# sunchao/leveldb-rs

Hardware: AMD Instinct MI355X
Metric: GiB/s device-resident batched CRC32C, 4KiB blocks; %HBM-peak at 1/2/4/8 GPUs (higher is better)
Workload: dtype u32

## Files before the change

leveldb-rs_amd/csrc/blocks.hip:

```cpp
#include <hip/hip_runtime.h>

#include <algorithm>
#include <string>

#include "lvh.h"

namespace lvk {

template <int G, bool STRIDED>
__global__ __launch_bounds__(kThreads) void crc32c_batch_kernel(Params P, const uint4 *__restrict__ image) {
    if (static_cast<uint64_t>(blockIdx.x) * kWaves * (64 / G) >= P.n) return;
    stage_tables(image);
    const uint32_t lane = threadIdx.x & 63u;
    const uint32_t wave = threadIdx.x >> 6;
    const Lut L = make_lut(lane);
    constexpr uint32_t kGroups = 64 / G;
    const uint64_t gid = (static_cast<uint64_t>(blockIdx.x) * kWaves + wave) * kGroups + lane / G;
    const uint64_t gstride = static_cast<uint64_t>(gridDim.x) * kWaves * kGroups;
    group_stream<G, STRIDED>(P, gid, gstride, lane % G, L);
}

constexpr uint32_t kFuseMax = 16;

__device__ __forceinline__ void fuse_pieces(const Params &P, const uint32_t *fm, uint32_t (&res)[kWaves][64],
                                            uint32_t lane, uint32_t wave) {
    __syncthreads();
    if (wave != 0) return;
    const uint32_t s = 1u << P.pshift;
    const uint64_t v = static_cast<uint64_t>(blockIdx.x) * 64u + lane;
    const uint32_t k = lane & (s - 1u);
    uint32_t acc = v < P.n ? gf2_apply(fm + (s - 1u - k) * 33u, res[lane >> 2][lane & 3u]) : 0u;
    for (uint32_t d = s >> 1; d >= 1; d >>= 1) acc ^= __shfl_xor(acc, d);
    if (v < P.n && k == 0) P.out[v >> P.pshift] = final_crc(P, acc);
}
static_assert(kFuseMax * 33 <= kWaves * 64, "fused combine matrices fit g_oidx");
template <int G, bool SEEDED, bool PIECES = false, bool FUSE = false, bool GATHER = false>
__global__ __launch_bounds__(kThreads) void crc32c_blocks_kernel(Params P, uint32_t nb,
                                                                 const uint4 *__restrict__ image) {
    static_assert(!FUSE || (PIECES && G == 16), "fused combine: pieces of the G = 16 kernel");
    const uint32_t lane = threadIdx.x & 63u;
    const uint32_t wave = __builtin_amdgcn_readfirstlane(threadIdx.x >> 6);
    constexpr uint32_t kGroups = 64 / G;
    constexpr uint64_t kRow = 16ull * G;
    constexpr uint64_t kBatch = kRow * U;
    const uint32_t gl = lane % G;
    constexpr uint32_t kW = kWaves;
    uint64_t blk = (static_cast<uint64_t>(blockIdx.x) * kW + wave) * kGroups + lane / G;
    const uint64_t gstride = static_cast<uint64_t>(gridDim.x) * kW * kGroups;
    const uint64_t wblk0 = (static_cast<uint64_t>(blockIdx.x) * kW + wave) * kGroups;
    const uint64_t pmask = (1ull << P.pshift) - 1;
    auto block_off = [&](uint64_t k) -> uint64_t {
        const uint64_t kk = k < P.n ? k : 0;
        const uint64_t b = PIECES ? kk >> P.pshift : kk;
        if constexpr (GATHER) return P.off[b];
        return b * P.stride;
    };
    auto report = [&](uint32_t bad) {
        if constexpr (GATHER)
            if (bad && P.herr) atomicOr(P.herr, bad);
    };
    auto block_at = [&](uint64_t k, uint64_t bo) {
        const uint64_t kk = k < P.n ? k : 0;
        if constexpr (GATHER) bo &= ~static_cast<uint64_t>(15);
        if constexpr (PIECES) return P.base + bo + (kk & pmask) * P.plen + 16u * gl;
        return P.base + bo + 16u * gl;
    };
    auto block_ptr = [&](uint64_t k) { return block_at(k, block_off(k)); };
    auto seed_ld = [&](uint64_t k) -> uint32_t {
        const uint64_t kk = k < P.n ? k : 0;
        if constexpr (PIECES) {
            const uint32_t sd = SEEDED ? ~P.seed[kk >> P.pshift] : 0xffffffffu;
            return (kk & pmask) ? 0u : sd;
        }
        return ~P.seed[kk];
    };
    constexpr bool kVarS0 = SEEDED || PIECES;

    const uint64_t o0 = block_off(blk);
    uint64_t ptr = block_at(blk, o0);
    uint64_t o1 = GATHER ? block_off(blk + gstride) : 0;
    uint64_t o2 = o1;
    uint32_t s0 = kVarS0 ? seed_ld(blk) : 0xffffffffu;
    uint32_t s0n = s0;
    uint4 slot0[U], slot1[U];
#pragma unroll
    for (uint32_t i = 0; i < U; ++i) slot0[i] = load16(ptr + kRow * i);
    const uint64_t nblk = PIECES ? (P.n >> P.pshift) : P.n;
    const uint64_t lstr = static_cast<uint64_t>(gridDim.x) * kThreads;
    const uint64_t lb0 = static_cast<uint64_t>(blockIdx.x) * kThreads + threadIdx.x;
    uint32_t lq[4] = {0, 0, 0, 0};
    const bool lcheck = GATHER && P.herr;
    if (lcheck) {
#pragma unroll
        for (uint32_t i = 0; i < 4; ++i) {
            const uint64_t b = lb0 + i * lstr;
            lq[i] = b < nblk ? P.len[b] ^ P.hlen : 0u;
        }
    }
    uint32_t *const fm = &g_oidx[0][0];
    if constexpr (FUSE) {
        const uint32_t nw = (1u << P.pshift) * 32u;
        for (uint32_t i = threadIdx.x; i < nw; i += kThreads) fm[(i >> 5) * 33 + (i & 31u)] = P.mats[i];
    }
    stage_tables(image);
    uint32_t lbad = lq[0] | lq[1] | lq[2] | lq[3];
    if (lcheck)
        for (uint64_t b = lb0 + 4 * lstr; b < nblk; b += lstr) lbad |= P.len[b] ^ P.hlen;
    if constexpr (GATHER) report(((o0 & 15u) ? LV_HINT_ERR_MISALIGNED : 0u) | (lbad ? LV_HINT_ERR_NOT_UNIFORM : 0u));
    if (wblk0 >= P.n) {
        if constexpr (FUSE) fuse_pieces(P, fm, g_ocrc, lane, wave);
        return;
    }
    if constexpr (PIECES) {
        if (nb <= U && (FUSE || wblk0 + gstride >= P.n)) {
            uint4 v1[U], v2[U], v3[U];
#pragma unroll
            for (uint32_t i = 0; i < U; ++i) {
                v1[i] = load16(ptr + kBatch * (nb > 1 ? 1u : 0u) + kRow * i);
                v2[i] = load16(ptr + kBatch * (nb > 2 ? 2u : 0u) + kRow * i);
                v3[i] = load16(ptr + kBatch * (nb > 3 ? 3u : 0u) + kRow * i);
            }
            const Lut L = make_lut(lane);
            uint32_t A[U];
            if (gl == 0) slot0[0].x ^= kVarS0 ? seed_ld(blk) : 0xffffffffu;
            fold_batch<true>(slot0, A, L);
            if (nb > 1) fold_batch<false>(v1, A, L);
            if (nb > 2) fold_batch<false>(v2, A, L);
            if (nb > 3) fold_batch<false>(v3, A, L);
            const uint32_t X = merge_group<G, -1, -1, true>(A, L);
            if constexpr (FUSE) {
                if (gl == 0) g_ocrc[wave][lane / G] = X;
                fuse_pieces(P, fm, g_ocrc, lane, wave);
            } else {
                if (gl == 0 && blk < P.n) P.out[blk] = X;
            }
            return;
        }
    }
    const uint64_t rounds = (P.n - 1 - wblk0) / gstride + 1;
    if (G == 16 && nb >= 8 && rounds * nb >= 64)
        for (uint32_t k = 0; k < wave * LVK_STAGGER; ++k) __builtin_amdgcn_s_sleep(32);
    const Lut L = make_lut(lane);
    uint32_t A[U];
    uint32_t st_val = 0;
    uint64_t st_ptr = 0;

    auto step = [&](uint64_t r, uint32_t j, uint4(&cur)[U], uint4(&nxt)[U]) {
        const bool lastj = j + 1 == nb;
        const bool more = !lastj || r + 1 < rounds;
        if constexpr (GATHER) o2 = block_off(blk + 2 * gstride);
        const uint64_t nptr = lastj ? (GATHER ? block_at(blk + gstride, o1) : block_ptr(blk + gstride)) : ptr + kBatch;
        const uint64_t lptr = more ? nptr : GATHER ? ptr : P.base + 16u * gl;
        if constexpr (kVarS0) s0n = seed_ld(blk + gstride);
#pragma unroll
        for (uint32_t i = 0; i < U; ++i) nxt[i] = load16(lptr + kRow * i);
        if (j == 0) {
            if (gl == 0) cur[0].x ^= s0;
            fold_batch<true>(cur, A, L);
        } else {
            fold_batch<false>(cur, A, L);
        }
        if (lastj) {
            const uint32_t X = merge_group<G, -1, -1, true>(A, L);
            if (gl == 0) g_ocrc[wave][(r % G) * kGroups + lane / G] = PIECES ? X : final_crc(P, X);
            if (!FUSE && ((r + 1) % G == 0 || r + 1 == rounds)) {
                __builtin_amdgcn_wave_barrier();
                const uint64_t r0 = r - r % G;
                const uint64_t k = wblk0 + (r0 + lane / kGroups) * gstride + lane % kGroups;
                st_val = g_ocrc[wave][lane];
                st_ptr = reinterpret_cast<uint64_t>(P.out + (k < P.n ? k : 0));
                if (lane < (r - r0 + 1) * kGroups && k < P.n) *reinterpret_cast<uint32_t *>(st_ptr) = st_val;
                __builtin_amdgcn_wave_barrier();
            }
            blk += gstride;
            if constexpr (kVarS0) s0 = s0n;
            if constexpr (GATHER) {
                if (o1 & 15u) report(LV_HINT_ERR_MISALIGNED);
                o1 = o2;
            }
        }
        ptr = nptr;
    };

    const uint64_t total = rounds * nb;
    uint64_t t = 0;
    uint64_t r = 0;
    uint32_t j = 0;
    for (;;) {
        step(r, j, slot0, slot1);
        if (++t == total) break;
        if (++j == nb) { j = 0; ++r; }
        step(r, j, slot1, slot0);
        if (++t == total) break;
        if (++j == nb) { j = 0; ++r; }
    }
    asm volatile("" ::"v"(st_val), "v"(st_ptr));
    if constexpr (FUSE) fuse_pieces(P, fm, g_ocrc, lane, wave);
}

__global__ __launch_bounds__(256) void combine_pieces_kernel(const uint32_t *__restrict__ raw, uint64_t n, uint32_t s,
                                                             const uint32_t *__restrict__ mats,
                                                             uint32_t *__restrict__ out, uint32_t flags) {
    __shared__ uint32_t M[65 * 33];
    for (uint32_t i = threadIdx.x; i < 65 * 32; i += blockDim.x) M[(i >> 5) * 33 + (i & 31u)] = mats[i];
    __syncthreads();
    const uint32_t lane = threadIdx.x & 63u;
    const uint32_t w = s < 64 ? s : 64, reps = s <= 64 ? 1 : s / 64;
    const uint64_t nw = static_cast<uint64_t>(gridDim.x) * (blockDim.x / 64);
    for (uint64_t b = static_cast<uint64_t>(blockIdx.x) * (blockDim.x / 64) + (threadIdx.x >> 6); b < n; b += nw) {
        uint32_t acc = 0;
        if (lane < w) {
            uint32_t nx = raw[b * s + lane];
            for (uint32_t m = 0; m < reps; ++m) {
                const uint32_t cur = nx;
                if (m + 1 < reps) nx = raw[b * s + lane + 64 * (m + 1)];
                acc = (m ? gf2_apply(M + 64 * 33, acc) : 0u) ^ cur;
            }
            acc = gf2_apply(M + (w - 1 - lane) * 33, acc);
        }
#pragma unroll
        for (int k = 32; k >= 1; k >>= 1) acc ^= __shfl_xor(acc, k);
        if (lane == 0) {
            const uint32_t crc = ~acc;
            out[b] = (flags & LV_CRC_MASK) ? mask_crc(crc) : crc;
        }
    }
}

__global__ __launch_bounds__(1024) void combine_pieces_wg_kernel(const uint32_t *__restrict__ raw, uint32_t s,
                                                                 const uint32_t *__restrict__ tabs,
                                                                 uint32_t *__restrict__ out, uint32_t flags) {
    __shared__ __attribute__((aligned(16))) uint32_t T[11 * 1024];
    __shared__ uint32_t part[16];
    const uint32_t c = s / 1024u;
    const uint32_t lc = c >= 4u ? 2u : 1u;
    stage_words(T, tabs, 256u);
    stage_words(T + 1024, tabs + lc * 1024u, 10u * 256u);
    __syncthreads();
    const uint32_t t = threadIdx.x, lane = t & 63u, w = t >> 6;
    const uint64_t b = blockIdx.x;
    uint32_t acc = 0;
    for (uint32_t i = 0; i < c; ++i) acc = (i ? tab_shift(T, acc) : 0u) ^ raw[b * s + t * c + i];
#pragma unroll
    for (uint32_t u = 0; u < 6; ++u) {
        const uint32_t right = __shfl_down(acc, 1u << u);
        const uint32_t sh = tab_shift(T + (1u + u) * 1024u, acc);
        if ((lane & ((2u << u) - 1u)) == 0) acc = sh ^ right;
    }
    if (lane == 0) part[w] = acc;
    __syncthreads();
    if (w == 0) {
        acc = lane < 16u ? part[lane] : 0u;
#pragma unroll
        for (uint32_t u = 0; u < 4; ++u) {
            const uint32_t right = __shfl_down(acc, 1u << u);
            const uint32_t sh = tab_shift(T + (7u + u) * 1024u, acc);
            if ((lane & ((2u << u) - 1u)) == 0) acc = sh ^ right;
        }
        if (lane == 0) {
            const uint32_t crc = ~acc;
            out[b] = (flags & LV_CRC_MASK) ? mask_crc(crc) : crc;
        }
    }
}

}

namespace lvh {

template <int G, bool STRIDED>
void launch_one(const DevCtx &c, int gi, const uint8_t *arena, const uint64_t *off,
                const uint32_t *len, uint64_t stride, uint32_t blen, const uint32_t *seed,
                uint32_t *out, uint64_t n, uint32_t flags, hipStream_t s) {
    const uint64_t groups_per_wg = static_cast<uint64_t>(lvk::kWaves) * (64 / G);
    uint64_t grid = (n + groups_per_wg - 1) / groups_per_wg;
    if (grid > static_cast<uint64_t>(c.cus)) grid = c.cus;
    if (grid == 0) grid = 1;
    lvk::Params P{};
    P.base = reinterpret_cast<uint64_t>(arena);
    P.off = off;
    P.len = len;
    P.seed = seed;
    P.out = out;
    P.n = n;
    P.stride = stride;
    P.blen = blen;
    P.flags = flags;
    P.ent = nullptr;
    P.sseed = nullptr;
    static const std::string name = std::string("crc32c_batch_kernel<") + std::to_string(G) +
                                    (STRIDED ? ",strided>" : ",offsets>");
    g_kernel = name.c_str();
    hipLaunchKernelGGL((lvk::crc32c_batch_kernel<G, STRIDED>), dim3(static_cast<uint32_t>(grid)),
                       dim3(lvk::kThreads), 0, s, P, c.image[gi]);
}

template <bool STRIDED>
void launch_g(const DevCtx &c, int gi, const uint8_t *arena, const uint64_t *off,
              const uint32_t *len, uint64_t stride, uint32_t blen, const uint32_t *seed,
              uint32_t *out, uint64_t n, uint32_t flags, hipStream_t s) {
    switch (gi) {
        case 0: launch_one<1, STRIDED>(c, gi, arena, off, len, stride, blen, seed, out, n, flags, s); break;
        case 1: launch_one<4, STRIDED>(c, gi, arena, off, len, stride, blen, seed, out, n, flags, s); break;
        case 2: launch_one<16, STRIDED>(c, gi, arena, off, len, stride, blen, seed, out, n, flags, s); break;
        default: launch_one<64, STRIDED>(c, gi, arena, off, len, stride, blen, seed, out, n, flags, s); break;
    }
}

void launch_group(const DevCtx &c, bool strided, int gi, const uint8_t *arena, const uint64_t *off,
                  const uint32_t *len, uint64_t stride, uint32_t blen, const uint32_t *seed, uint32_t *out, uint64_t n,
                  uint32_t flags, hipStream_t s) {
    if (strided)
        launch_g<true>(c, gi, arena, off, len, stride, blen, seed, out, n, flags, s);
    else
        launch_g<false>(c, gi, arena, off, len, stride, blen, seed, out, n, flags, s);
}

uint32_t pick_split(uint64_t base, uint64_t stride, uint64_t blen, uint64_t n, int forced, int cus) {
    if (forced >= 0 || base % 16 || stride % 16) return 0;
    const uint64_t want = 4ull * static_cast<uint64_t>(cus) * lvk::kWaves;
    uint32_t ps = 0;
    while ((n << ps) < want && ps < 12) {
        const uint64_t s2 = 2ull << ps;
        if (blen % s2 || (blen / s2) % 1024 || blen / s2 < 4096) break;
        ++ps;
    }
    return ps;
}
int pick_block_gi(uint64_t base, uint64_t stride, uint64_t blen, int forced, uint64_t n, int cus) {
    if (blen == 0 || base % 16 || stride % 16) return -1;
    auto fits = [&](int gi) { return blen % (16ull * kGs[gi] * lvk::U) == 0; };
    if (forced >= 0) return fits(forced) ? forced : -1;
    if (n < 4ull * static_cast<uint64_t>(cus) * lvk::kWaves && fits(3)) return 3;
    for (int gi : {2, 1, 0})
        if (fits(gi)) return gi;
    return -1;
}

template <int G, bool GATHER>
void launch_blocks_g(const DevCtx &c, int gi, const uint8_t *base, uint64_t stride, const uint64_t *off,
                     const uint32_t *len, const HintCheck *hc, uint32_t blen, uint64_t n, const uint32_t *seed,
                     uint32_t *out, uint32_t flags, hipStream_t s) {
    const uint64_t groups_per_wg = static_cast<uint64_t>(lvk::kWaves) * (64 / G);
    uint64_t grid = (n + groups_per_wg - 1) / groups_per_wg;
    if (grid > static_cast<uint64_t>(c.cus)) grid = c.cus;
    if (grid == 0) grid = 1;
    lvk::Params P{};
    P.base = reinterpret_cast<uint64_t>(base);
    P.off = off;
    P.len = len;
    P.seed = seed;
    P.out = out;
    P.n = n;
    P.stride = stride;
    P.blen = blen;
    P.flags = flags;
    P.ent = nullptr;
    P.sseed = nullptr;
    set_hint(P, hc, blen);
    const uint32_t nb = static_cast<uint32_t>(blen / (16ull * G * lvk::U));
    static const std::string name = "crc32c_blocks_kernel<" + std::to_string(G) + (GATHER ? ",gather>" : ">");
    g_kernel = name.c_str();
    if (seed)
        hipLaunchKernelGGL((lvk::crc32c_blocks_kernel<G, true, false, false, GATHER>),
                           dim3(static_cast<uint32_t>(grid)), dim3(lvk::kThreads), 0, s, P, nb, c.image[gi]);
    else
        hipLaunchKernelGGL((lvk::crc32c_blocks_kernel<G, false, false, false, GATHER>),
                           dim3(static_cast<uint32_t>(grid)), dim3(lvk::kThreads), 0, s, P, nb, c.image[gi]);
}

template <bool GATHER>
void launch_blocks(const DevCtx &c, int gi, const uint8_t *base, uint64_t stride, const uint64_t *off,
                   const uint32_t *len, const HintCheck *hc, uint32_t blen, uint64_t n, const uint32_t *seed,
                   uint32_t *out, uint32_t flags, hipStream_t s) {
    switch (gi) {
        case 0: launch_blocks_g<1, GATHER>(c, gi, base, stride, off, len, hc, blen, n, seed, out, flags, s); break;
        case 1: launch_blocks_g<4, GATHER>(c, gi, base, stride, off, len, hc, blen, n, seed, out, flags, s); break;
        case 2: launch_blocks_g<16, GATHER>(c, gi, base, stride, off, len, hc, blen, n, seed, out, flags, s); break;
        default: launch_blocks_g<64, GATHER>(c, gi, base, stride, off, len, hc, blen, n, seed, out, flags, s); break;
    }
}

template <bool GATHER>
void launch_pieces(DevCtx &c, uint32_t ps, const uint32_t *mats, const uint32_t *tabs, const uint8_t *base,
                   uint64_t stride, const uint64_t *off, const uint32_t *len, const HintCheck *hc, uint32_t blen,
                   uint64_t n, const uint32_t *seed, uint32_t *out, uint32_t flags, hipStream_t hs, uint32_t *scr) {
    const uint64_t nv = n << ps, plen = blen >> ps;
    const uint32_t nb = static_cast<uint32_t>(plen / (16ull * 16 * lvk::U));
    lvk::Params P{};
    P.base = reinterpret_cast<uint64_t>(base);
    P.off = off;
    P.len = len;
    P.seed = seed;
    P.n = nv;
    P.stride = stride;
    P.blen = static_cast<uint32_t>(plen);
    P.flags = flags;
    P.plen = plen;
    P.pshift = ps;
    P.mats = mats;
    set_hint(P, hc, blen);
    if (!scr) {
        P.out = out;
        const dim3 grid(static_cast<uint32_t>((nv + 63) / 64));
        if (seed)
            hipLaunchKernelGGL((lvk::crc32c_blocks_kernel<16, true, true, true, GATHER>), grid, dim3(lvk::kThreads), 0,
                               hs, P, nb, c.image[2]);
        else
            hipLaunchKernelGGL((lvk::crc32c_blocks_kernel<16, false, true, true, GATHER>), grid, dim3(lvk::kThreads),
                               0, hs, P, nb, c.image[2]);
        g_kernel = GATHER ? "crc32c_blocks_kernel<16,pieces,fused,gather>" : "crc32c_blocks_kernel<16,pieces,fused>";
        return;
    }
    P.out = scr;
    const uint64_t grid = std::min<uint64_t>(c.cus, (nv + 63) / 64);
    if (seed)
        hipLaunchKernelGGL((lvk::crc32c_blocks_kernel<16, true, true, false, GATHER>), dim3(static_cast<uint32_t>(grid)),
                           dim3(lvk::kThreads), 0, hs, P, nb, c.image[2]);
    else
        hipLaunchKernelGGL((lvk::crc32c_blocks_kernel<16, false, true, false, GATHER>),
                           dim3(static_cast<uint32_t>(grid)), dim3(lvk::kThreads), 0, hs, P, nb, c.image[2]);
    if (ps >= 11) {
        hipLaunchKernelGGL(lvk::combine_pieces_wg_kernel, dim3(static_cast<uint32_t>(n)), dim3(1024), 0, hs, P.out,
                           1u << ps, tabs, out, flags);
        g_kernel = GATHER ? "crc32c_blocks_kernel<16,pieces,gather>+combine_pieces_wg_kernel"
                          : "crc32c_blocks_kernel<16,pieces>+combine_pieces_wg_kernel";
    } else {
        hipLaunchKernelGGL(lvk::combine_pieces_kernel, dim3(static_cast<uint32_t>(std::min<uint64_t>(1024, (n + 3) / 4))),
                           dim3(256), 0, hs, P.out, n, 1u << ps, mats, out, flags);
        g_kernel = GATHER ? "crc32c_blocks_kernel<16,pieces,gather>+combine_pieces_kernel"
                          : "crc32c_blocks_kernel<16,pieces>+combine_pieces_kernel";
    }
}

UniformPlan uniform_plan(int cus, uint64_t base, uint64_t stride, uint32_t blen, uint64_t n, int gi) {
    UniformPlan pl{};
    pl.ps = pick_split(base, stride, blen, n, gi, cus);
    pl.bgi = -1;
    if (pl.ps > 0) {
        const uint64_t nv = n << pl.ps;
        const bool fused = (1u << pl.ps) <= lvk::kFuseMax && nv <= 64ull * static_cast<uint64_t>(cus);
        pl.scratch = fused ? 0 : nv * 4;
    } else {
        pl.bgi = pick_block_gi(base, stride, blen, gi, n, cus);
    }
    return pl;
}

int launch_uniform(DevCtx &c, const UniformPlan &pl, const uint8_t *base, uint64_t stride, const uint64_t *off,
                   const uint32_t *len, const HintCheck *hc, uint32_t blen, uint64_t n, const uint32_t *seed,
                   uint32_t *out, uint32_t flags, hipStream_t hs, uint8_t *scr) {
    if (pl.ps > 0) {
        const uint64_t plen = blen >> pl.ps;
        const uint32_t *mats = nullptr, *tabs = nullptr;
        if (int rc = piece_mats(c, plen, &mats)) return rc;
        if (pl.scratch && pl.ps >= 11)
            if (int rc = piece_tabs(c, plen, &tabs)) return rc;
        uint32_t *s32 = pl.scratch ? reinterpret_cast<uint32_t *>(scr) : nullptr;
        if (off)
            launch_pieces<true>(c, pl.ps, mats, tabs, base, stride, off, len, hc, blen, n, seed, out, flags, hs, s32);
        else
            launch_pieces<false>(c, pl.ps, mats, tabs, base, stride, off, len, hc, blen, n, seed, out, flags, hs,
                                 s32);
        return 0;
    }
    if (off)
        launch_blocks<true>(c, pl.bgi, base, stride, off, len, hc, blen, n, seed, out, flags, hs);
    else
        launch_blocks<false>(c, pl.bgi, base, stride, off, len, hc, blen, n, seed, out, flags, hs);
    return 0;
}

}

using namespace lvh;

extern "C" {

int lv_crc32c_batch_strided(const uint8_t *d_base, uint64_t stride, uint32_t block_len, size_t n,
                            const uint32_t *d_seed, uint32_t *d_out, uint32_t flags, void *stream) {
    g_err.clear();
    if (n == 0) return LV_OK;
    if (!d_base || !d_out) return set_err(LV_ERR_INVALID, "null device pointer");
    if (n > 0xffffffffull) return set_err(LV_ERR_INVALID, "more than 2^32-1 buffers per call");
    DevCtx *c = nullptr;
    if (int rc = current_ctx(&c)) return rc;
    const int gi = forced_gi(flags);
    hipStream_t hs = static_cast<hipStream_t>(stream);
    const UniformPlan pl = uniform_plan(c->cus, reinterpret_cast<uint64_t>(d_base), stride, block_len, n, gi);
    if (pl.applies()) {
        uint8_t *scr = nullptr;
        std::unique_lock<std::mutex> ws_lk;
        if (pl.scratch)
            if (int rc = stream_ws_bytes(*c, hs, pl.scratch, &scr, &ws_lk)) return rc;
        if (int rc = launch_uniform(*c, pl, d_base, stride, nullptr, nullptr, nullptr, block_len, n, d_seed, d_out,
                                    flags, hs, scr))
            return rc;
        return check_launch();
    }
    launch_g<true>(*c, gi >= 0 ? gi : pick_gi(block_len), d_base, nullptr, nullptr, stride, block_len, d_seed,
                   d_out, n, flags, hs);
    return check_launch();
}

}
```

leveldb-rs_amd/csrc/context.hip:

```cpp
#include <hip/hip_runtime.h>

#include <algorithm>
#include <cstring>
#include <thread>

#include "../../include/lvgpu/crc32c.h"
#include "crc32c_gf2.h"
#include "lvh.h"

namespace lvk {

__device__ __forceinline__ uint64_t splitmix64(uint64_t x) {
    x += 0x9E3779B97F4A7C15ull;
    x = (x ^ (x >> 30)) * 0xBF58476D1CE4E5B9ull;
    x = (x ^ (x >> 27)) * 0x94D049BB133111EBull;
    return x ^ (x >> 31);
}

__global__ void fill_words_kernel(uint64_t *dst, uint64_t word0, uint64_t nwords, uint64_t seed) {
    for (uint64_t i = blockIdx.x * 256ull + threadIdx.x; i < nwords; i += gridDim.x * 256ull)
        dst[i] = splitmix64(seed ^ (word0 + i));
}

__global__ void fill_bytes_kernel(uint8_t *dst, uint64_t begin, uint64_t nbytes, uint64_t seed) {
    for (uint64_t i = blockIdx.x * 256ull + threadIdx.x; i < nbytes; i += gridDim.x * 256ull) {
        const uint64_t k = begin + i;
        dst[i] = static_cast<uint8_t>(splitmix64(seed ^ (k >> 3)) >> (8 * (k & 7)));
    }
}

}

namespace lvh {

thread_local std::string g_err;
thread_local const char *g_kernel = "";

int set_err(int code, const std::string &msg) {
    g_err = msg;
    return code;
}

const std::vector<uint32_t> &host_image(int gi) {
    static std::vector<uint32_t> images[kImages];
    static std::once_flag once;
    std::call_once(once, [] {
        uint32_t T[4][256], C[6][4][256];
        lvgpu::slice_tables(T);
        for (int k = 0; k < 6; ++k) lvgpu::shift_tables(16ull << k, C[k]);
        for (int i = 0; i < 4; ++i) {
            const uint64_t G = static_cast<uint64_t>(kGs[i]);
            uint32_t W4[4][256], W1[4][256], W2[4][256];
            lvgpu::shift_tables(16ull * G * lvk::U, W4);
            lvgpu::shift_tables(16ull * G, W1);
            lvgpu::shift_tables(32ull * G, W2);
            std::vector<uint32_t> &im = images[i];
            im.assign(lvk::kImageWords, 0u);
            uint32_t *ra = &im[lvk::kRegionA / 4], *rb = &im[lvk::kRegionB / 4];
            for (int e = 0; e < 256; ++e)
                for (int c = 0; c < 8; ++c)
                    for (int k = 0; k < 4; ++k) {
                        ra[e * 64 + 4 * c + k] = T[k][e];
                        ra[e * 64 + 32 + 4 * c + k] = W4[3 - k][e];
                        rb[e * 64 + 4 * c + k] = W1[3 - k][e];
                        rb[e * 64 + 32 + 4 * c + k] = W2[3 - k][e];
                    }
            uint32_t *rc = &im[lvk::kComb / 4];
            for (int k = 0; k < 6; ++k)
                for (int j = 0; j < 4; ++j)
                    for (int e = 0; e < 256; ++e) rc[(k * 4 + j) * 256 + e] = C[k][j][e];
        }
        uint32_t WT[4][256];
        lvgpu::shift_tables(256ull * lvk::kSstRows, WT);
        images[kTableImage] = images[2];
        uint32_t *ra = &images[kTableImage][lvk::kRegionA / 4];
        for (int e = 0; e < 256; ++e)
            for (int c = 0; c < 8; ++c)
                for (int k = 0; k < 4; ++k) ra[e * 64 + 32 + 4 * c + k] = WT[3 - k][e];
    });
    return images[gi];
}

DevCounters g_count[64];

DevCounters &counters() {
    int d = 0;
    if (hipGetDevice(&d) != hipSuccess || d < 0 || d >= 64) d = 0;
    return g_count[d];
}

int grow_dev(uint8_t **p, size_t *cap, size_t need) {
    if (*cap >= need) return 0;
    if (*p) LV_HIP(hipFree(*p));
    *p = nullptr;
    *cap = 0;
    LV_HIP(hipMalloc(p, need));
    counters().allocs++;
    *cap = need;
    return 0;
}

int grow_pinned(uint8_t **p, size_t *cap, size_t need) {
    if (*cap >= need) return 0;
    if (*p) LV_HIP(hipHostFree(*p));
    *p = nullptr;
    *cap = 0;
    LV_HIP(hipHostMalloc(p, need, hipHostMallocDefault));
    counters().allocs++;
    *cap = need;
    return 0;
}

bool is_pinned(const void *p) {
    hipPointerAttribute_t a;
    const hipError_t e = hipPointerGetAttributes(&a, p);
    if (e != hipSuccess) {
        (void)hipGetLastError();
        return false;
    }
    return a.type == hipMemoryTypeHost;
}

void par_memcpy(uint8_t *dst, const uint8_t *src, size_t bytes, unsigned threads) {
    unsigned nt = std::thread::hardware_concurrency();
    nt = nt == 0 ? 1 : (nt > threads ? threads : nt);
    if (bytes < (4u << 20) || nt == 1) {
        std::memcpy(dst, src, bytes);
        return;
    }
    std::vector<std::thread> th;
    const size_t per = (bytes + nt - 1) / nt;
    for (unsigned t = 0; t < nt; ++t) {
        const size_t lo = t * per;
        if (lo >= bytes) break;
        const size_t len = bytes - lo < per ? bytes - lo : per;
        th.emplace_back([=] { std::memcpy(dst + lo, src + lo, len); });
    }
    for (auto &x : th) x.join();
}

DevCtx g_dev[64];

int current_ctx(DevCtx **out) {
    int dev = 0;
    hipError_t e = hipGetDevice(&dev);
    if (e != hipSuccess) return set_err(LV_ERR_NO_DEVICE, std::string("hipGetDevice: ") + hipGetErrorString(e));
    if (dev < 0 || dev >= 64) return set_err(LV_ERR_NO_DEVICE, "device index out of range");
    DevCtx &c = g_dev[dev];
    std::lock_guard<std::mutex> lk(c.m);
    if (!c.ready) {
        hipDeviceProp_t prop;
        LV_HIP(hipGetDeviceProperties(&prop, dev));
        c.cus = prop.multiProcessorCount;
        for (int i = 0; i < kImages; ++i) {
            const auto &im = host_image(i);
            LV_HIP(hipMalloc(&c.image[i], im.size() * 4));
            counters().allocs++;
            LV_HIP(hipMemcpy(c.image[i], im.data(), im.size() * 4, hipMemcpyHostToDevice));
        }
        {
            std::vector<uint32_t> bt(lvk::kBaseMats * 1024);
            for (uint32_t i = 0; i < lvk::kBaseMats; ++i) {
                uint32_t S[4][256];
                lvgpu::shift_tables(1ull << i, S);
                for (int j = 0; j < 4; ++j)
                    for (int e = 0; e < 256; ++e) bt[i * 1024 + j * 256 + e] = S[j][e];
            }
            LV_HIP(hipMalloc(&c.base_tabs, bt.size() * 4));
            counters().allocs++;
            LV_HIP(hipMemcpy(c.base_tabs, bt.data(), bt.size() * 4, hipMemcpyHostToDevice));
        }
        c.ready = true;
    }
    *out = &c;
    return 0;
}

int pick_gi(uint64_t len) {
    if (len <= 128) return 0;
    if (len <= 1024) return 1;
    if (len <= 16384) return 2;
    return 3;
}

int forced_gi(uint32_t flags) {
    const uint32_t f = (flags & LV_CRC_GROUP_MASK) >> 8;
    return f ? static_cast<int>(f) - 1 : -1;
}

static StreamWs *find_ws(DevCtx &c, hipStream_t s, bool create) {
    std::lock_guard<std::mutex> mk(c.ws_m);
    if (!create) {
        auto it = c.ws.find(s);
        return it == c.ws.end() ? nullptr : it->second.get();
    }
    auto &slot = c.ws[s];
    if (!slot) slot.reset(new StreamWs);
    return slot.get();
}

int stream_ws_bytes(DevCtx &c, hipStream_t s, size_t need, uint8_t **out, std::unique_lock<std::mutex> *lk) {
    StreamWs *w = find_ws(c, s, true);
    *lk = std::unique_lock<std::mutex>(w->m);
    if (w->cap < need) {
        if (w->p) LV_HIP(hipFree(w->p));
        w->p = nullptr;
        w->cap = 0;
        LV_HIP(hipMalloc(&w->p, need));
        counters().allocs++;
        w->cap = need;
    }
    *out = w->p;
    return 0;
}

int stream_ws(DevCtx &c, hipStream_t s, uint64_t n, uint8_t **out, std::unique_lock<std::mutex> *lk) {
    return stream_ws_bytes(c, s, sort_ws_bytes(n), out, lk);
}

int stream_err(DevCtx &c, hipStream_t s, uint32_t **out) {
    StreamWs *w = find_ws(c, s, true);
    std::lock_guard<std::mutex> lk(w->em);
    if (!w->err) {
        LV_HIP(hipHostMalloc(reinterpret_cast<void **>(&w->herr), 4, hipHostMallocDefault));
        LV_HIP(hipMalloc(&w->err, 4));
        counters().allocs += 2;
        LV_HIP(hipMemsetAsync(w->err, 0, 4, s));
    }
    *out = w->err;
    return 0;
}
// ... 339 lines not shown
```

leveldb-rs_amd/csrc/lvh.h:

```cpp
#pragma once
#include <hip/hip_runtime.h>

#include <atomic>
#include <cstdint>
#include <map>
#include <memory>
#include <mutex>
#include <string>
#include <vector>

#include "../../include/lvgpu/crc32c.h"
#include "lv_internal.h"
#include "lvk/core.h"

namespace lvh {

extern thread_local std::string g_err;
extern thread_local const char *g_kernel;
int set_err(int code, const std::string &msg);

#define LV_HIP(call)                                                                   \
    do {                                                                               \
        hipError_t e_ = (call);                                                        \
        if (e_ != hipSuccess)                                                          \
            return set_err(static_cast<int>(e_), std::string(#call) + ": " +           \
                                                     hipGetErrorString(e_));           \
    } while (0)


constexpr int kGs[4] = {1, 4, 16, 64};
constexpr int kTableImage = 4;
constexpr uint32_t kAlRowsH = LVK_AL_ROWS;
constexpr int kAlImage = kAlRowsH == 4 ? 2 : kTableImage;
static_assert(kAlRowsH == 4 || kAlRowsH == lvk::kSstRows, "aligned rows: 4, or the table image's");
constexpr int kImages = 5;

const std::vector<uint32_t> &host_image(int gi);

struct StreamWs {
    std::mutex m;
    uint8_t *p = nullptr;
    size_t cap = 0;
    std::mutex em;
    uint32_t *err = nullptr;
    uint32_t *herr = nullptr;
};

struct DevCtx {
    std::mutex m;
    bool ready = false;
    int cus = 0;
    uint4 *image[kImages] = {};
    uint32_t *base_tabs = nullptr;
    std::mutex ws_m;
    std::map<hipStream_t, std::unique_ptr<StreamWs>> ws;
    std::mutex mats_m;
    std::map<uint64_t, uint32_t *> piece_mats;
    std::map<uint64_t, uint32_t *> piece_tabs;
    std::mutex host_m;
    uint8_t *d_arena = nullptr;
    size_t d_arena_cap = 0;
    uint8_t *d_meta = nullptr;
    size_t d_meta_cap = 0;
    uint8_t *h_meta = nullptr;
    size_t h_meta_cap = 0;
    uint8_t *h_stage[2] = {nullptr, nullptr};
    size_t h_stage_cap[2] = {0, 0};
    hipEvent_t ev[2] = {nullptr, nullptr};
    hipStream_t stream = nullptr;
    hipStream_t stream2 = nullptr;
    uint8_t *d_arena2 = nullptr;
    size_t d_arena2_cap = 0;
    uint8_t *d_scr[2] = {nullptr, nullptr};
    size_t d_scr_cap[2] = {0, 0};
    int dev = 0;
};

constexpr size_t kStageBytes = 64ull << 20;

struct DevCounters {
    std::atomic<uint64_t> h2d{0}, d2h{0}, allocs{0};
};
extern DevCounters g_count[64];
DevCounters &counters();


int grow_dev(uint8_t **p, size_t *cap, size_t need);
int grow_pinned(uint8_t **p, size_t *cap, size_t need);
bool is_pinned(const void *p);
void par_memcpy(uint8_t *dst, const uint8_t *src, size_t bytes, unsigned threads = LVK_MEMCPY_THREADS);
int current_ctx(DevCtx **out);
int pick_gi(uint64_t len);
int forced_gi(uint32_t flags);
int check_launch();

constexpr size_t al16(size_t x) { return (x + 15) & ~static_cast<size_t>(15); }

inline bool overlaps(const void *a, uint64_t ab, const void *b, uint64_t bb) {
    const uintptr_t x = reinterpret_cast<uintptr_t>(a), y = reinterpret_cast<uintptr_t>(b);
    return ab && bb && x < y + bb && y < x + ab;
}
inline bool misaligned(const void *p, uintptr_t n) { return reinterpret_cast<uintptr_t>(p) % n != 0; }

struct Carve {
    uint8_t *base;
    size_t at = 0;
    template <class T>
    T *take(size_t count) {
        const size_t o = at;
        at += al16(count * sizeof(T));
        return base ? reinterpret_cast<T *>(reinterpret_cast<uintptr_t>(base) + o) : nullptr;
    }
};

uint64_t sort_wgs(uint64_t n, uint64_t *chunk);
struct WsLayout {
    size_t m, wgb, ent, sseed, part, longs, tmp, pos, total;
};
WsLayout ws_layout(uint64_t n);
size_t sort_ws_bytes(uint64_t n);
int stream_ws_bytes(DevCtx &c, hipStream_t s, size_t need, uint8_t **out, std::unique_lock<std::mutex> *lk);
int stream_ws(DevCtx &c, hipStream_t s, uint64_t n, uint8_t **out, std::unique_lock<std::mutex> *lk);
int piece_mats(DevCtx &c, uint64_t plen, const uint32_t **out);
int piece_tabs(DevCtx &c, uint64_t plen, const uint32_t **out);

struct HintCheck {
    uint32_t *err;
    uint64_t total;
    uint32_t len;
    uint32_t uniform;
};
inline void set_hint(lvk::Params &P, const HintCheck *hc, uint32_t dflt_len) {
    P.herr = hc ? hc->err : nullptr;
    P.htotal = hc ? hc->total : 0;
    P.hlen = hc ? hc->len : dflt_len;
    P.huni = hc ? hc->uniform : 0;
}
int stream_err(DevCtx &c, hipStream_t s, uint32_t **out);
int check_hints(hipStream_t s, uint32_t *violations);

uint4 *launch_sort(uint8_t *ws_bytes, const uint64_t *off, const uint32_t *len, const uint32_t *seed, uint64_t n,
                   hipStream_t s, lvk::Params *P);
void launch_sort_scan(uint32_t *M, uint32_t wgs, uint32_t *ws, uint64_t *wgb, hipStream_t s);
int launch_binned(DevCtx &c, uint8_t *ws_bytes, const uint8_t *arena, const uint64_t *off, const uint32_t *len,
                  const uint32_t *seed, uint32_t *out, uint64_t n, uint32_t flags, hipStream_t s, bool join = true,
                  const HintCheck *hc = nullptr);
bool hint_needs_join(const lv_batch_hint &h, uint64_t n, uint32_t cus);
void launch_classes(const DevCtx &c, bool seeded, const lvk::Params &P, const uint32_t *ws, hipStream_t s);
void launch_group(const DevCtx &c, bool strided, int gi, const uint8_t *arena, const uint64_t *off,
                  const uint32_t *len, uint64_t stride, uint32_t blen, const uint32_t *seed, uint32_t *out, uint64_t n,
                  uint32_t flags, hipStream_t s);
struct UniformPlan {
    uint32_t ps;
    int bgi;
    uint64_t scratch;
    bool applies() const { return ps > 0 || bgi >= 0; }
};
UniformPlan uniform_plan(int cus, uint64_t base, uint64_t stride, uint32_t blen, uint64_t n, int gi);
int launch_uniform(DevCtx &c, const UniformPlan &pl, const uint8_t *base, uint64_t stride, const uint64_t *off,
                   const uint32_t *len, const HintCheck *hc, uint32_t blen, uint64_t n, const uint32_t *seed,
                   uint32_t *out, uint32_t flags, hipStream_t hs, uint8_t *scr);

}
```

leveldb-rs_amd/csrc/lvk/core.h:

```cpp
#pragma once
#include <hip/hip_runtime.h>

#include <cstdint>

#include "../../../include/lvgpu/crc32c.h"
#include "knobs.h"

namespace lvk {

constexpr int kThreads = 1024;
constexpr int kWaves = kThreads / 64;
constexpr uint32_t U = 4;

constexpr uint32_t kRegionA = 0;
constexpr uint32_t kRegionB = 65536;
constexpr uint32_t kHalf = 128;
constexpr uint32_t kComb = 131072;
constexpr int kImageWords = (131072 + 6 * 4 * 1024) / 4;

static __shared__ __attribute__((aligned(16))) uint32_t g_lds[kImageWords];

static __shared__ uint32_t g_oidx[kWaves][64];
static __shared__ uint32_t g_ocrc[kWaves][64];
static_assert(sizeof(uint32_t) * (kImageWords + 2 * kWaves * 64) <= 163840, "LDS budget");

struct Lut {
    uint32_t lv, sel0, sel1, sel2, sel3;
};

__device__ __forceinline__ Lut make_lut(uint32_t lane) {
    const uint32_t g = lane & 31u, c = g & 7u, q = g >> 3;
    Lut L;
    L.lv = 0;
    uint32_t sel[4];
#pragma unroll
    for (uint32_t i = 0; i < 4; ++i) {
        const uint32_t k = (q + i) & 3u;
        L.lv |= ((4u * c + k) * 4u) << (8u * i);
        sel[i] = 0x0C0C0000u | ((4u + 3u - k) << 8) | i;
    }
    L.sel0 = sel[0];
    L.sel1 = sel[1];
    L.sel2 = sel[2];
    L.sel3 = sel[3];
    return L;
}

__device__ __forceinline__ uint32_t lds_word(uint32_t byte_addr) {
    return *reinterpret_cast<const uint32_t *>(reinterpret_cast<const char *>(g_lds) + byte_addr);
}

__device__ __forceinline__ uint32_t xor3(uint32_t a, uint32_t b, uint32_t c) {
    return __builtin_amdgcn_bitop3_b32(a, b, c, 0x96);
}

template <uint32_t OFF>
__device__ __forceinline__ uint32_t lookup4(uint32_t s, const Lut &L) {
    const uint32_t a0 = __builtin_amdgcn_perm(s, L.lv, L.sel0);
    const uint32_t a1 = __builtin_amdgcn_perm(s, L.lv, L.sel1);
    const uint32_t a2 = __builtin_amdgcn_perm(s, L.lv, L.sel2);
    const uint32_t a3 = __builtin_amdgcn_perm(s, L.lv, L.sel3);
    return xor3(lds_word(a0 + OFF), lds_word(a1 + OFF), lds_word(a2 + OFF)) ^ lds_word(a3 + OFF);
}

template <uint32_t OFF>
__device__ __forceinline__ uint32_t lookup4x(uint32_t s, uint32_t x, const Lut &L) {
    const uint32_t a0 = __builtin_amdgcn_perm(s, L.lv, L.sel0);
    const uint32_t a1 = __builtin_amdgcn_perm(s, L.lv, L.sel1);
    const uint32_t a2 = __builtin_amdgcn_perm(s, L.lv, L.sel2);
    const uint32_t a3 = __builtin_amdgcn_perm(s, L.lv, L.sel3);
    return xor3(xor3(lds_word(a0 + OFF), lds_word(a1 + OFF), lds_word(a2 + OFF)), lds_word(a3 + OFF), x);
}

__device__ __forceinline__ uint32_t r0_granule(uint4 v, const Lut &L) {
    uint32_t s = lookup4x<kRegionA>(v.x, v.y, L);
    s = lookup4x<kRegionA>(s, v.z, L);
    s = lookup4x<kRegionA>(s, v.w, L);
    return lookup4<kRegionA>(s, L);
}

template <int I>
__device__ __forceinline__ uint32_t lut_addr(uint32_t s, const Lut &L) {
    const uint32_t sel = I == 0 ? L.sel0 : I == 1 ? L.sel1 : I == 2 ? L.sel2 : L.sel3;
    return __builtin_amdgcn_perm(s, L.lv, sel);
}

__device__ __forceinline__ uint32_t comb_shift(uint32_t a, int k) {
    const uint32_t *t = g_lds + (kComb / 4) + k * 1024;
    return t[a & 0xffu] ^ t[256 + ((a >> 8) & 0xffu)] ^ t[512 + ((a >> 16) & 0xffu)] ^
           t[768 + (a >> 24)];
}

template <bool FIRST, int W4K = -1, uint32_t NU = U, uint32_t W4OFF = kRegionA + kHalf, uint32_t SKIP = 0>
__device__ __forceinline__ void fold_batch(const uint4 (&v)[NU], uint32_t (&A)[NU], const Lut &L) {
    static_assert(SKIP == 0 || FIRST, "only a first batch skips rows");
    static_assert(SKIP < NU, "at least one row");
    uint32_t s[NU], w[NU], w3[NU];
#pragma unroll
    for (uint32_t i = 0; i < NU; ++i) s[i] = v[i].x;
    if constexpr (SKIP > 0) {
#pragma unroll
        for (uint32_t i = 0; i < SKIP; ++i) A[i] = 0u;
    }
    if constexpr (!FIRST && W4K >= 0) {
#pragma unroll
        for (uint32_t i = 0; i < NU; ++i) {
            w[i] = comb_shift(A[i], W4K);
            w3[i] = 0u;
        }
    } else if constexpr (!FIRST) {
        uint32_t aa[NU][4];
#pragma unroll
        for (uint32_t i = 0; i < NU; ++i) {
            aa[i][0] = lut_addr<0>(A[i], L);
            aa[i][1] = lut_addr<1>(A[i], L);
            aa[i][2] = lut_addr<2>(A[i], L);
            aa[i][3] = lut_addr<3>(A[i], L);
        }
#pragma unroll
        for (uint32_t i = 0; i < NU; ++i) {
            w[i] = xor3(lds_word(aa[i][0] + W4OFF), lds_word(aa[i][1] + W4OFF),
                        lds_word(aa[i][2] + W4OFF));
            w3[i] = lds_word(aa[i][3] + W4OFF);
        }
    }
#pragma unroll
    for (uint32_t step = 0; step < 4; ++step) {
        uint32_t ad[NU][4];
#pragma unroll
        for (uint32_t i = SKIP; i < NU; ++i) {
            ad[i][0] = lut_addr<0>(s[i], L);
            ad[i][1] = lut_addr<1>(s[i], L);
            ad[i][2] = lut_addr<2>(s[i], L);
            ad[i][3] = lut_addr<3>(s[i], L);
        }
        uint32_t t[NU][4];
#pragma unroll
        for (uint32_t i = SKIP; i < NU; ++i)
#pragma unroll
            for (uint32_t k = 0; k < 4; ++k) t[i][k] = lds_word(ad[i][k] + kRegionA);
#pragma unroll
        for (uint32_t i = SKIP; i < NU; ++i) {
            const uint32_t x = xor3(t[i][0], t[i][1], t[i][2]);
            if (step < 3) {
                const uint32_t nw = step == 0 ? v[i].y : step == 1 ? v[i].z : v[i].w;
                s[i] = xor3(x, t[i][3], nw);
            } else if constexpr (FIRST) {
                A[i] = x ^ t[i][3];
            } else {
                A[i] = x ^ xor3(t[i][3], w[i], w3[i]);
            }
        }
    }
}


__device__ __forceinline__ uint32_t byte_step(uint32_t s, uint32_t b) {
    const uint32_t c4 = (__lane_id() & 7u) * 4u;
    const uint32_t e = (s ^ b) & 0xffu;
    return g_lds[e * 64u + c4] ^ (s >> 8);
}

__device__ __forceinline__ uint32_t fix_word(uint32_t w, int32_t rel, uint32_t s0) {
    const int32_t z = -rel;
    const uint32_t keep = z <= 0 ? 0xffffffffu : (z >= 4 ? 0u : 0xffffffffu << (8 * z));
    const uint32_t sx =
        (rel >= 4 || rel <= -4) ? 0u : (rel >= 0 ? s0 >> (8 * rel) : s0 << (8 * z));
    return (w & keep) ^ sx;
}

typedef uint32_t u32x4 __attribute__((ext_vector_type(4)));
typedef const __attribute__((address_space(1))) u32x4 g_u32x4;

__device__ __forceinline__ uint4 to_uint4(u32x4 v) { return make_uint4(v.x, v.y, v.z, v.w); }

__device__ __forceinline__ uint4 load16(uint64_t addr) {
    return to_uint4(__builtin_nontemporal_load(reinterpret_cast<g_u32x4 *>(addr)));
}

__device__ __forceinline__ uint4 load16_rt(uint64_t addr) {
    return to_uint4(*reinterpret_cast<g_u32x4 *>(addr));
}

template <uint32_t I>
__device__ __forceinline__ uint4 load_row(uint64_t addr) {
    if constexpr (I == U - 1) return load16_rt(addr);
    return load16(addr);
}

__device__ __forceinline__ uint32_t mask_crc(uint32_t c) {
    return ((c >> 15) | (c << 17)) + 0xa282ead8u;
}

struct Params {
    uint64_t base;
    const uint64_t *off;
    const uint32_t *len;
    const uint32_t *seed;
    uint32_t *out;
    uint64_t n;
    uint64_t stride;
    uint32_t blen;
    uint32_t flags;
    uint64_t plen;
    uint32_t pshift;
    const uint4 *ent;
    const uint32_t *sseed;
    uint64_t nplain;
    uint32_t *part;
    uint32_t *tmp;
    const uint32_t *mats;
    const uint32_t *tabs;
    uint32_t hident;
    uint32_t *herr;
    uint64_t htotal;
    uint32_t hlen;
    uint32_t huni;
};

struct Geo {
    uint64_t abase;
    uint32_t bid;
    uint32_t len;
    uint32_t seed;
    uint32_t nb;
    int32_t hoff;
    uint32_t alow;
};

template <int G>
__device__ __forceinline__ Geo make_geo(uint64_t a, uint32_t len, uint32_t seed) {
    constexpr int32_t GU = G * static_cast<int32_t>(U);
    Geo q;
    q.abase = a & ~static_cast<uint64_t>(15);
    q.len = len;
    q.seed = seed;
    const uint32_t alow = static_cast<uint32_t>(a & 15u);
    const int32_t ng = static_cast<int32_t>(((alow + len) >> 4));
    const int32_t nb = ng > 0 ? (ng + GU - 1) / GU : 1;
    q.nb = static_cast<uint32_t>(nb);
    q.hoff = ng - GU * nb;
    const bool fix2 = nb > 1 && q.hoff == -(GU - 1) && alow > 12u;
    q.alow = alow | (fix2 ? 16u : 0u);
    return q;
}

template <int G, bool STRIDED>
__device__ __forceinline__ Geo fetch_geo(const Params &P, uint64_t i) {
    Geo q;
    uint64_t b = i;
    if constexpr (STRIDED) {
        q = make_geo<G>(P.base + b * P.stride, P.blen, P.seed ? P.seed[b] : 0u);
    } else if (P.ent) {
        const uint4 e = P.ent[i];
        b = e.w;
        q = make_geo<G>(P.base + ((static_cast<uint64_t>(e.y) << 32) | e.x), e.z, P.seed ? P.seed[b] : 0u);
    } else {
        q = make_geo<G>(P.base + P.off[b], P.len[b], P.seed ? P.seed[b] : 0u);
    }
    q.bid = static_cast<uint32_t>(b);
    return q;
}

template <int G>
__device__ __forceinline__ void load_batch(const Geo &q, uint32_t j, uint32_t gl, uint4 (&v)[U]) {
    const int32_t d = q.hoff + static_cast<int32_t>(G * U * j + gl);
    const uint64_t p = q.abase + (static_cast<int64_t>(d) << 4);
    v[0] = load_row<0>(p);
    v[1] = load_row<1>(p + 16u * G);
    v[2] = load_row<2>(p + 32u * G);
    v[3] = load_row<3>(p + 48u * G);
}

template <int G>
__device__ __forceinline__ void load_batch0(const Geo &q, uint32_t gl, uint4 (&v)[U]) {
#pragma unroll
    for (uint32_t i = 0; i < U; ++i) {
        int32_t d = q.hoff + static_cast<int32_t>(G * i + gl);
        d = d < 0 ? 0 : d;
        const uint64_t a = q.abase + (static_cast<uint32_t>(d) << 4);
        v[i] = i == U - 1 ? load16_rt(a) : load16(a);
    }
}

__device__ __forceinline__ uint4 load_tail(const Geo &q, uint32_t gl) {
    const uint32_t end = (q.alow & 15u) + q.len;
    if (gl == 0 && (end & 15u)) return load16(q.abase + (end & ~15u));
    return make_uint4(0, 0, 0, 0);
}

template <int G>
__device__ __forceinline__ void fix_head(const Geo &q, uint32_t j, uint32_t gl, uint4 (&v)[U]) {
    const uint32_t s0 = q.len >= 4 ? ~q.seed : 0u;
    const int32_t alow = static_cast<int32_t>(q.alow & 15u);
#pragma unroll
    for (uint32_t i = 0; i < U; ++i) {
        const int32_t d = q.hoff + static_cast<int32_t>(G * (U * j + i) + gl);
        if (d == 0 || (d == 1 && alow > 12)) {
            const int32_t rel = d * 16 - alow;
            v[i].x = fix_word(v[i].x, rel, s0);
            v[i].y = fix_word(v[i].y, rel + 4, s0);
            v[i].z = fix_word(v[i].z, rel + 8, s0);
            v[i].w = fix_word(v[i].w, rel + 12, s0);
        }
    }
}

template <int G>
// ... 208 lines not shown
```

Before: 6074.

## Carry the CRC state across batches with a precomputed shift table instead of re-folding

Replaces the fold_batch first/rest variants with a fold_batch_carry routine. It XORs the running accumulator into the first word of each batch. On non-final batches its last step uses a second table region, which holds shift tables for the batch stride, to advance the state across the remaining distance. New per-group LDS images with those jump tables are built on the host and passed to the blocks and pieces kernels. The aim is to drop the extra xor terms and table lookups (w, w3) in the non-first fold path, at the cost of more host images and a per-step choice of lookup tables.

Result: faster. 6199, median of 6 (+2.1%).

```diff
diff --git a/leveldb-rs_amd/csrc/blocks.hip b/leveldb-rs_amd/csrc/blocks.hip
--- a/leveldb-rs_amd/csrc/blocks.hip
+++ b/leveldb-rs_amd/csrc/blocks.hip
@@ -121,12 +121,12 @@
                 v3[i] = load16(ptr + kBatch * (nb > 3 ? 3u : 0u) + kRow * i);
             }
             const Lut L = make_lut(lane);
-            uint32_t A[U];
+            uint32_t A[U] = {};
             if (gl == 0) slot0[0].x ^= kVarS0 ? seed_ld(blk) : 0xffffffffu;
-            fold_batch<true>(slot0, A, L);
-            if (nb > 1) fold_batch<false>(v1, A, L);
-            if (nb > 2) fold_batch<false>(v2, A, L);
-            if (nb > 3) fold_batch<false>(v3, A, L);
+            fold_batch_carry(slot0, A, L, nb == 1);
+            if (nb > 1) fold_batch_carry(v1, A, L, nb == 2);
+            if (nb > 2) fold_batch_carry(v2, A, L, nb == 3);
+            if (nb > 3) fold_batch_carry(v3, A, L, nb == 4);
             const uint32_t X = merge_group<G, -1, -1, true>(A, L);
             if constexpr (FUSE) {
                 if (gl == 0) g_ocrc[wave][lane / G] = X;
@@ -141,7 +141,7 @@
     if (G == 16 && nb >= 8 && rounds * nb >= 64)
         for (uint32_t k = 0; k < wave * LVK_STAGGER; ++k) __builtin_amdgcn_s_sleep(32);
     const Lut L = make_lut(lane);
-    uint32_t A[U];
+    uint32_t A[U] = {};
     uint32_t st_val = 0;
     uint64_t st_ptr = 0;
 
@@ -154,14 +154,12 @@
         if constexpr (kVarS0) s0n = seed_ld(blk + gstride);
 #pragma unroll
         for (uint32_t i = 0; i < U; ++i) nxt[i] = load16(lptr + kRow * i);
-        if (j == 0) {
-            if (gl == 0) cur[0].x ^= s0;
-            fold_batch<true>(cur, A, L);
-        } else {
-            fold_batch<false>(cur, A, L);
-        }
+        if (j == 0 && gl == 0) cur[0].x ^= s0;
+        fold_batch_carry(cur, A, L, lastj);
         if (lastj) {
             const uint32_t X = merge_group<G, -1, -1, true>(A, L);
+#pragma unroll
+            for (uint32_t i = 0; i < U; ++i) A[i] = 0u;
             if (gl == 0) g_ocrc[wave][(r % G) * kGroups + lane / G] = PIECES ? X : final_crc(P, X);
             if (!FUSE && ((r + 1) % G == 0 || r + 1 == rounds)) {
                 __builtin_amdgcn_wave_barrier();
@@ -361,12 +359,13 @@
     const uint32_t nb = static_cast<uint32_t>(blen / (16ull * G * lvk::U));
     static const std::string name = "crc32c_blocks_kernel<" + std::to_string(G) + (GATHER ? ",gather>" : ">");
     g_kernel = name.c_str();
+    const uint4 *image = c.image[kBlocksImage + gi];
     if (seed)
         hipLaunchKernelGGL((lvk::crc32c_blocks_kernel<G, true, false, false, GATHER>),
-                           dim3(static_cast<uint32_t>(grid)), dim3(lvk::kThreads), 0, s, P, nb, c.image[gi]);
+                           dim3(static_cast<uint32_t>(grid)), dim3(lvk::kThreads), 0, s, P, nb, image);
     else
         hipLaunchKernelGGL((lvk::crc32c_blocks_kernel<G, false, false, false, GATHER>),
-                           dim3(static_cast<uint32_t>(grid)), dim3(lvk::kThreads), 0, s, P, nb, c.image[gi]);
+                           dim3(static_cast<uint32_t>(grid)), dim3(lvk::kThreads), 0, s, P, nb, image);
 }
 
 template <bool GATHER>
@@ -400,15 +399,16 @@
     P.pshift = ps;
     P.mats = mats;
     set_hint(P, hc, blen);
+    const uint4 *image = c.image[kBlocksImage + 2];
     if (!scr) {
         P.out = out;
         const dim3 grid(static_cast<uint32_t>((nv + 63) / 64));
         if (seed)
             hipLaunchKernelGGL((lvk::crc32c_blocks_kernel<16, true, true, true, GATHER>), grid, dim3(lvk::kThreads), 0,
-                               hs, P, nb, c.image[2]);
+                               hs, P, nb, image);
         else
             hipLaunchKernelGGL((lvk::crc32c_blocks_kernel<16, false, true, true, GATHER>), grid, dim3(lvk::kThreads),
-                               0, hs, P, nb, c.image[2]);
+                               0, hs, P, nb, image);
         g_kernel = GATHER ? "crc32c_blocks_kernel<16,pieces,fused,gather>" : "crc32c_blocks_kernel<16,pieces,fused>";
         return;
     }
@@ -416,10 +416,10 @@
     const uint64_t grid = std::min<uint64_t>(c.cus, (nv + 63) / 64);
     if (seed)
         hipLaunchKernelGGL((lvk::crc32c_blocks_kernel<16, true, true, false, GATHER>), dim3(static_cast<uint32_t>(grid)),
-                           dim3(lvk::kThreads), 0, hs, P, nb, c.image[2]);
+                           dim3(lvk::kThreads), 0, hs, P, nb, image);
     else
         hipLaunchKernelGGL((lvk::crc32c_blocks_kernel<16, false, true, false, GATHER>),
-                           dim3(static_cast<uint32_t>(grid)), dim3(lvk::kThreads), 0, hs, P, nb, c.image[2]);
+                           dim3(static_cast<uint32_t>(grid)), dim3(lvk::kThreads), 0, hs, P, nb, image);
     if (ps >= 11) {
         hipLaunchKernelGGL(lvk::combine_pieces_wg_kernel, dim3(static_cast<uint32_t>(n)), dim3(1024), 0, hs, P.out,
                            1u << ps, tabs, out, flags);
diff --git a/leveldb-rs_amd/csrc/context.hip b/leveldb-rs_amd/csrc/context.hip
--- a/leveldb-rs_amd/csrc/context.hip
+++ b/leveldb-rs_amd/csrc/context.hip
@@ -77,6 +77,15 @@
         for (int e = 0; e < 256; ++e)
             for (int c = 0; c < 8; ++c)
                 for (int k = 0; k < 4; ++k) ra[e * 64 + 32 + 4 * c + k] = WT[3 - k][e];
+        for (int i = 0; i < 4; ++i) {
+            uint32_t J[4][256];
+            lvgpu::shift_tables(16ull * kGs[i] * lvk::U - 12, J);
+            images[kBlocksImage + i] = images[i];
+            uint32_t *rj = &images[kBlocksImage + i][lvk::kRegionA / 4];
+            for (int e = 0; e < 256; ++e)
+                for (int c = 0; c < 8; ++c)
+                    for (int k = 0; k < 4; ++k) rj[e * 64 + 32 + 4 * c + k] = J[3 - k][e];
+        }
     });
     return images[gi];
 }
diff --git a/leveldb-rs_amd/csrc/lvh.h b/leveldb-rs_amd/csrc/lvh.h
--- a/leveldb-rs_amd/csrc/lvh.h
+++ b/leveldb-rs_amd/csrc/lvh.h
@@ -33,7 +33,8 @@
 constexpr uint32_t kAlRowsH = LVK_AL_ROWS;
 constexpr int kAlImage = kAlRowsH == 4 ? 2 : kTableImage;
 static_assert(kAlRowsH == 4 || kAlRowsH == lvk::kSstRows, "aligned rows: 4, or the table image's");
-constexpr int kImages = 5;
+constexpr int kBlocksImage = 5;
+constexpr int kImages = 9;
 
 const std::vector<uint32_t> &host_image(int gi);
 
diff --git a/leveldb-rs_amd/csrc/lvk/core.h b/leveldb-rs_amd/csrc/lvk/core.h
--- a/leveldb-rs_amd/csrc/lvk/core.h
+++ b/leveldb-rs_amd/csrc/lvk/core.h
@@ -154,6 +154,41 @@
     }
 }
 
+template <uint32_t NU = U>
+__device__ __forceinline__ void fold_batch_carry(const uint4 (&v)[NU], uint32_t (&A)[NU], const Lut &L, bool last) {
+    Lut L3 = L;
+    L3.lv = last ? L.lv : L.lv | 0x80808080u;
+    uint32_t s[NU];
+#pragma unroll
+    for (uint32_t i = 0; i < NU; ++i) s[i] = v[i].x ^ A[i];
+#pragma unroll
+    for (uint32_t step = 0; step < 4; ++step) {
+        const Lut &Ls = step < 3 ? L : L3;
+        uint32_t ad[NU][4];
+#pragma unroll
+        for (uint32_t i = 0; i < NU; ++i) {
+            ad[i][0] = lut_addr<0>(s[i], Ls);
+            ad[i][1] = lut_addr<1>(s[i], Ls);
+            ad[i][2] = lut_addr<2>(s[i], Ls);
+            ad[i][3] = lut_addr<3>(s[i], Ls);
+        }
+        uint32_t t[NU][4];
+#pragma unroll
+        for (uint32_t i = 0; i < NU; ++i)
+#pragma unroll
+            for (uint32_t k = 0; k < 4; ++k) t[i][k] = lds_word(ad[i][k] + kRegionA);
+#pragma unroll
+        for (uint32_t i = 0; i < NU; ++i) {
+            const uint32_t x = xor3(t[i][0], t[i][1], t[i][2]);
+            if (step < 3) {
+                const uint32_t nw = step == 0 ? v[i].y : step == 1 ? v[i].z : v[i].w;
+                s[i] = xor3(x, t[i][3], nw);
+            } else {
+                A[i] = x ^ t[i][3];
+            }
+        }
+    }
+}
 
 __device__ __forceinline__ uint32_t byte_step(uint32_t s, uint32_t b) {
     const uint32_t c4 = (__lane_id() & 7u) * 4u;
```
